# open-genome/dna

Measured on AMD Instinct MI355X. Metric: MLM sequences/sec, DNABERT-2-117M seq_len=512, at 1/2/4/8 MI355X, higher is better.
Workload: dtype bf16

## Files before the change

dna_amd/_native.py:

```python
import ctypes
import os
import re

import torch

_HERE = os.path.dirname(os.path.abspath(__file__))
LIB_PATH = os.environ.get("DNA_AMD_LIB", os.path.join(_HERE, "lib", "libdna_amd.so"))
HEADER = os.path.join(os.path.dirname(_HERE), "include", "dna_amd.h")

F32, BF16, F16 = 0, 1, 2
ACT_NONE, ACT_GELU, ACT_SIGMOID = 0, 1, 2
DCONV_PLAIN, DCONV_GATE, DCONV_MAIN_MUL, DCONV_MAIN_ADD = 0, 1, 2, 3
CLS_REGRESSION, CLS_SINGLE_LABEL, CLS_MULTI_LABEL = 0, 1, 2

_vp, _i, _u64, _f, _sz = ctypes.c_void_p, ctypes.c_int, ctypes.c_uint64, ctypes.c_float, ctypes.c_size_t
_i64 = ctypes.c_int64

_SIGS = {
    "dna_abi_version": (_i, []),
    "dna_abi_revision": (_i, []),
    "dna_last_error": (ctypes.c_char_p, []),
    "dna_attn_fwd": (_i, [_vp, _vp, _vp, _i, _i, _i, _i, _i, _f, _vp, _vp, _vp]),
    "dna_attn_bwd": (_i, [_vp, _vp, _vp, _vp, _vp, _vp, _i, _i, _i, _i, _i, _f, _vp, _vp, _vp]),
    "dna_attn_bwd_ex": (_i, [_vp, _vp, _vp, _vp, _vp, _vp, _i, _i, _i, _i, _i, _f, _vp, _vp, _vp, _vp]),
    "dna_attn_bwd_var": (_i, [_vp, _vp, _vp, _vp, _vp, _vp, _i, _i, _i, _i, _i, _f, _vp, _vp, _vp, _i, _vp]),
    "dna_attn_dbias_part_rows": (_i, [_i, _i]),
    "dna_attn_varlen_fwd": (_i, [_vp, _vp, _vp, _vp, _i, _i, _i, _i, _i, _i, _f, _vp, _vp, _vp]),
    "dna_attn_varlen_bwd_workspace": (_sz, [_i, _i, _i, _i]),
    "dna_attn_varlen_bwd": (_i, [_vp, _vp, _vp, _vp, _vp, _vp, _vp, _i, _i, _i, _i, _i, _i, _f, _vp,
                                 _vp, _vp]),
    "dna_flash_lse_rows": (_i, [_i]),
    "dna_flash_fwd": (_i, [_vp, _i, _vp, _i, _i, _i64, _i64, _i64, _i, _i, _i, _i, _i, _f, _vp, _vp, _vp]),
    "dna_flash_bwd": (_i, [_vp, _i, _vp, _i, _i, _i64, _i64, _i64, _vp, _vp, _vp, _i, _i, _i, _i, _i,
                           _f, _vp, _vp, _vp]),
    "dna_colsum_f32": (_i, [_vp, _i, _i, _vp, _i, _vp]),
    "dna_colsum_bf16_workspace": (_sz, [_i, _i]),
    "dna_colsum_bf16": (_i, [_vp, _i, _i, _vp, _i, _vp, _sz, _vp]),
    "dna_flip_rows": (_i, [_vp, _i, _i, _sz, _vp, _vp]),
    "dna_causal_conv1d_fwd": (_i, [_vp, _sz, _i, _vp, _vp, _i, _i, _i, _i, _i, _vp, _vp]),
    "dna_causal_conv1d_part_rows": (_sz, [_i, _i]),
    "dna_causal_conv1d_bwd": (_i, [_vp, _sz, _i, _vp, _vp, _vp, _i, _i, _i, _i, _i, _vp, _sz, _vp, _vp]),
    "dna_hyena_shortconv_fwd": (_i, [_vp, _i, _vp, _vp, _i, _i, _i, _i, _i, _vp, _vp, _vp]),
    "dna_hyena_shortconv_part_elems": (_sz, [_i, _i, _i, _i, _i]),
    "dna_hyena_shortconv_bwd": (_i, [_vp, _i, _vp, _vp, _i, _i, _i, _i, _i, _vp, _vp, _vp, _vp, _vp]),
    "dna_hyena_gate_out_fwd": (_i, [_vp, _vp, _i, _i, _i, _i, _sz, _vp, _vp]),
    "dna_hyena_gate_out_bwd": (_i, [_vp, _vp, _vp, _i, _i, _i, _i, _sz, _vp, _vp, _vp]),
    "dna_hyena_modulate_t_fwd": (_i, [_vp, _i, _vp, _vp, _f, _i, _i, _i, _vp, _vp]),
    "dna_hyena_modulate_t_bwd": (_i, [_vp, _vp, _vp, _f, _i, _i, _i, _vp, _i, _vp]),
    "dna_hyena_filter_part_elems": (_i, [_i, _i, _i, _i]),
    "dna_hyena_filter_part_stride": (_i, [_i, _i, _i]),
    "dna_hyena_filter_fwd": (_i, [_vp, _vp, _vp, _vp, _vp, _i, _vp, _vp, _vp, _vp, _f, _i, _i, _i, _i,
                                  _vp, _vp]),
    "dna_hyena_filter_bwd": (_i, [_vp, _vp, _vp, _vp, _vp, _i, _vp, _vp, _vp, _vp, _f, _i, _i, _i, _i,
                                  _vp, _vp, _vp, _vp]),
    "dna_hyena_filter_finish": (_i, [_vp, _i, _i, _i, _vp, _vp]),
    "dna_ln_fwd": (_i, [_vp, _i, _vp, _i, _f, _u64, _u64, _vp, _vp, _vp, _i, _i, _f, _vp, _vp,
                        _vp, _vp, _vp]),
    "dna_ln_bwd_workspace": (_sz, [_i, _i]),
    "dna_ln_bwd": (_i, [_vp, _vp, _vp, _i, _vp, _i, _f, _u64, _u64, _vp, _vp, _vp, _vp, _i, _i,
                        _vp, _vp, _vp, _vp, _vp, _vp, _sz, _vp]),
    "dna_ln_bwd_from_y": (_i, [_vp, _vp, _vp, _i, _f, _u64, _u64, _vp, _vp, _vp, _i, _i, _vp,
                               _vp, _vp, _vp, _vp, _vp, _sz, _vp]),
    "dna_ln_bwd_from_y_acc": (_i, [_vp, _vp, _vp, _i, _f, _u64, _u64, _vp, _vp, _vp, _i, _i, _vp,
                                   _vp, _vp, _vp, _vp, _vp, _sz, _vp]),
    "dna_ln_from_y_check": (_i, [_vp, _vp, _vp, _vp, _i, _f, _f, _f, _f, _vp, _vp]),
    "dna_add_ln_fwd": (_i, [_vp, _i, _vp, _vp, _vp, _i, _i, _f, _i, _vp, _vp, _vp, _vp, _vp, _vp]),
    "dna_add_ln_bwd": (_i, [_vp, _vp, _vp, _vp, _i, _vp, _vp, _vp, _vp, _i, _i, _i, _vp, _vp, _vp,
                            _vp, _vp, _sz, _vp]),
    "dna_rms_fwd": (_i, [_vp, _i, _vp, _i, _i, _f, _vp, _vp, _vp, _vp]),
    "dna_rms_bwd": (_i, [_vp, _vp, _vp, _i, _vp, _vp, _i, _i, _vp, _vp, _vp, _sz, _vp]),
    "dna_embed_ln_fwd": (_i, [_vp, _vp, _vp, _vp, _vp, _i, _i, _i, _f, _f, _u64, _u64, _vp, _vp,
                              _vp, _vp, _vp]),
    "dna_embed_ln_bwd": (_i, [_vp, _vp, _vp, _vp, _vp, _vp, _vp, _vp, _i, _i, _i, _i, _f, _u64,
                              _u64, _vp, _vp, _vp, _vp, _vp, _sz, _vp]),
    "dna_embed_ln_bwd_rows": (_i, [_vp, _vp, _vp, _vp, _vp, _vp, _vp, _vp, _i, _i, _i, _f, _u64,
                                   _u64, _vp, _vp, _vp, _vp, _vp, _sz, _vp]),
    "dna_embed_grad_segsum_workspace": (_sz, [_i, _i]),
    "dna_embed_grad_segsum": (_i, [_vp, _vp, _vp, _i, _i, _i, _i, _vp, _vp, _sz, _vp]),
    "dna_sum_slices_accum": (_i, [_vp, _i, _sz, _vp, _vp]),
    "dna_sum_slices": (_i, [_vp, _i, _sz, _vp, _vp]),
    "dna_geglu_fwd": (_i, [_vp, _i, _i, _i, _f, _u64, _u64, _vp, _vp, _vp]),
    "dna_geglu_bwd": (_i, [_vp, _vp, _i, _i, _i, _vp, _vp]),
    "dna_linear_fwd": (_i, [_vp, _vp, _vp, _i, _i, _i, _vp, _vp]),
# ... 146 lines not shown
```

dna_amd/bert_layers.py:

```python
import math
from dataclasses import dataclass
from typing import Optional, Tuple

import torch
import torch.nn as nn

from . import functional as DF
from .config import BertConfig, alibi_slopes

try:
    from transformers.modeling_outputs import MaskedLMOutput
except Exception:
    @dataclass
    class MaskedLMOutput:
        loss: Optional[torch.Tensor] = None
        logits: Optional[object] = None
        hidden_states: Optional[object] = None
        attentions: Optional[object] = None

        def __getitem__(self, i):
            return (self.loss, self.logits)[i]

try:
    from transformers.modeling_outputs import SequenceClassifierOutput
# ... 140 lines not shown
        return self._lpt_provider(p)

    def _linear(self, x, w, b=None, geglu=None):
        return DF.linear(x, w, self._lp(w), b, w_lpt=self._lp_t(w), geglu=geglu)

    def _check_inputs(self, input_ids, token_type_ids, attention_mask):
        if input_ids is None:
            raise ValueError("Must specify input_ids (inputs_embeds is not supported)")
        if token_type_ids is not None and bool((token_type_ids != 0).any()):
            raise NotImplementedError("token_type_ids other than 0 (the MLM path never sets them)")
        if attention_mask is not None:
            if not torch.equal(attention_mask.bool(), input_ids != self.config.pad_token_id_mask):
                raise NotImplementedError("attention_mask must equal input_ids != [PAD]")

    def encode(self, input_ids: torch.Tensor, last_rows: Optional[torch.Tensor] = None,
               packed: Optional["PackedIndex"] = None):
        cfg = self.config
        bert = self._bert_model()
        b, S0 = input_ids.shape
        bf16 = self.precision == "bf16"
        S = S0
        if packed is not None:
            packed.check(input_ids)
            input_ids = input_ids.reshape(-1).index_select(0, packed.indices)
            if last_rows is not None:
                last_rows = packed.row_of.index_select(0, last_rows)
        elif bf16 and S0 % 64:
            S = (S0 + 63) // 64 * 64
            input_ids = torch.nn.functional.pad(input_ids, (0, S - S0), value=cfg.pad_token_id_mask)
            if last_rows is not None:
                last_rows = torch.div(last_rows, S0, rounding_mode="floor") * S + last_rows % S0
        T = b * S if packed is None else packed.total
        H = cfg.num_attention_heads
        train = self.training
        rng = self.dropout_rng
        p_hidden = cfg.hidden_dropout_prob if train else 0.0
        if cfg.attention_probs_dropout_prob and train:
            raise NotImplementedError("attention-probability dropout (reference default 0.0)")
        eps = cfg.layer_norm_eps
        ids = input_ids.reshape(-1)
        key_valid = None if packed is not None else (ids != cfg.pad_token_id_mask).to(torch.uint8)

        emb = bert.embeddings
        seed, off = rng.take(T * cfg.hidden_size) if p_hidden else (0, 0)
        x32, xb = DF.EmbeddingLN.apply(ids, emb.word_embeddings.weight,
                                       emb.token_type_embeddings.weight, emb.LayerNorm.weight,
                                       emb.LayerNorm.bias, eps, p_hidden, seed, off, True, bf16)
        xin = xb if bf16 else x32
        slopes = bert.encoder.alibi_slopes
        L = len(bert.encoder.layer)
        for i, layer in enumerate(bert.encoder.layer):
            att = layer.attention
            qkv = self._linear(xin, att.self.Wqkv.weight, att.self.Wqkv.bias)
            if packed is not None:
                ctx = DF.alibi_attention_varlen(qkv, packed, slopes, H)
            else:
                ctx = DF.alibi_attention(qkv, key_valid, slopes, b, S, H,
                                         bias_grad=att.self.Wqkv.bias is not None)
            res = x32
            if i == L - 1 and last_rows is not None:
                ctx = ctx.index_select(0, last_rows)
                res = x32.index_select(0, last_rows)
            n = ctx.shape[0]
            out = att.output
            h = self._linear(ctx, out.dense.weight)
            seed, off = rng.take(n * cfg.hidden_size) if p_hidden else (0, 0)
            y32, yb = DF.FusedLayerNorm.apply(h, out.dense.bias, res, out.LayerNorm.weight,
                                              out.LayerNorm.bias, eps, 0, p_hidden, seed, off,
                                              True, bf16)
            mlp = layer.mlp
            seed, off = rng.take(n * cfg.intermediate_size) if p_hidden else (0, 0)
            g = self._linear(yb if bf16 else y32, mlp.gated_layers.weight,
                             geglu=(p_hidden, seed, off))
            wo_lp, wo_lpt = self._lp(mlp.wo.weight), self._lp_t(mlp.wo.weight)
            if DF.geglu_out_fused_ok(g, wo_lp, wo_lpt):
                o = DF.geglu_out(g, p_hidden, seed, off, mlp.wo.weight, wo_lp, wo_lpt)
            else:
                a = DF.GeGLU.apply(g, p_hidden, seed, off)
                o = DF.linear(a, mlp.wo.weight, wo_lp, None, w_lpt=wo_lpt)
            x32, xb = DF.FusedLayerNorm.apply(o, mlp.wo.bias, y32, mlp.layernorm.weight,
                                              mlp.layernorm.bias, eps, 0, 0.0, 0, 0, True, bf16)
            xin = xb if bf16 else x32
        if L == 0 and last_rows is not None:
            x32, xin = x32.index_select(0, last_rows), xin.index_select(0, last_rows)
        if packed is None and last_rows is None and S != S0:
            d = x32.shape[1]
            x32 = x32.view(b, S, d)[:, :S0].reshape(b * S0, d)
            xin = xin.view(b, S, d)[:, :S0].reshape(b * S0, d)
        return x32, xin


class BertModel(nn.Module, _HipEncoder):

    def __init__(self, config, add_pooling_layer=False, precision: str = "bf16",
                 init_weights: bool = True):
        super().__init__()
        config = BertConfig.from_any(config)
        self.config = config
        self.embeddings = BertEmbeddings(config)
        self.encoder = BertEncoder(config)
        self.pooler = BertPooler(config) if add_pooling_layer else None
        self._init_hip_encoder(precision)
        if init_weights:
            _init_bert_weights(self, config.initializer_range)
            _tag_projections(self.encoder)

    def _bert_model(self):
        return self

    def forward(self, input_ids, token_type_ids=None, attention_mask=None, position_ids=None,
                output_all_encoded_layers=False, masked_tokens_mask=None, packed=None, **kwargs):
        if output_all_encoded_layers or masked_tokens_mask is not None:
            raise NotImplementedError("BertModel.forward: last layer only, no masked_tokens_mask "
                                      "(the MLM subset path is BertForMaskedLM.mlm_logits)")
# ... 271 lines not shown
```

dna_amd/functional.py:

```python
import math
import os
import warnings

import torch
import torch.nn as nn
import torch.nn.functional as F

from . import _native as N
from .flat import raw_writes

_DT = {torch.float32: N.F32, torch.bfloat16: N.BF16}


def _dt(t):
    try:
        return _DT[t.dtype]
    except KeyError:
        raise TypeError(f"dna_amd: unsupported dtype {t.dtype} (fp32 / bf16 only)")


def _gpu(*ts):
    for t in ts:
        if t is not None and not t.is_cuda:
            raise RuntimeError("dna_amd ops run on the GPU only (no CPU fallback); "
# ... 521 lines not shown
                           + 2 * x.element_size()) + 4)
        with _timed("rms_bwd", nbytes, "byte"):
            N.call("dna_rms_bwd", _p(dy), _p(dyb), x.data_ptr(), _dt(x), gamma.data_ptr(),
                   rstd.data_ptr(), n, d, dx.data_ptr(), dg.data_ptr(), ws.data_ptr(), nws,
                   N.stream_ptr())
        return dx, dg, None, None, None


class AlibiAttention(torch.autograd.Function):

    @staticmethod
    def forward(ctx, qkv, key_valid, slopes, b, S, H, scale, bias_grad=False):
        _gpu(qkv, key_valid, slopes)
        qkv = qkv.contiguous()
        T = qkv.shape[0]
        D = qkv.shape[1] // (3 * H)
        out = torch.empty(T, H * D, device=qkv.device, dtype=qkv.dtype)
        lse = torch.empty(b, H, S, device=qkv.device, dtype=torch.float32)
        with _timed("attn_fwd", 4.0 * b * H * S * S * D):
            N.call("dna_attn_fwd", qkv.data_ptr(), _p(key_valid), slopes.data_ptr(), b, S, H, D,
                   _dt(qkv), scale, out.data_ptr(), lse.data_ptr(), N.stream_ptr())
        ctx.save_for_backward(qkv, out, lse, key_valid, slopes)
        ctx.cfg = (b, S, H, D, scale)
        ctx.bias_grad = bias_grad and qkv.dtype == torch.bfloat16
        return out

    @staticmethod
    def backward(ctx, dout):
        qkv, out, lse, key_valid, slopes = ctx.saved_tensors
        b, S, H, D, scale = ctx.cfg
        dqkv = torch.empty_like(qkv)
        delta = torch.empty(b * H * S, device=qkv.device, dtype=torch.float32)
        dout = dout.contiguous()
        part = None
        if ctx.bias_grad:
            rows = N.lib().dna_attn_dbias_part_rows(b, S)
            part = torch.empty(rows, qkv.shape[1], device=qkv.device, dtype=torch.float32)
        with _timed("attn_bwd", 10.0 * b * H * S * S * D):
            N.call("dna_attn_bwd_ex", qkv.data_ptr(), out.data_ptr(), dout.data_ptr(),
                   lse.data_ptr(), _p(key_valid), slopes.data_ptr(), b, S, H, D, _dt(qkv), scale,
                   dqkv.data_ptr(), delta.data_ptr(), _p(part), N.stream_ptr())
        if part is not None:
            colsum = torch.empty(qkv.shape[1], device=qkv.device, dtype=torch.float32)
            N.call("dna_colsum_f32", part.data_ptr(), part.shape[0], part.shape[1],
                   colsum.data_ptr(), 0, N.stream_ptr())
            dqkv._dna_colsum = colsum
        return dqkv, None, None, None, None, None, None, None


def alibi_attention(qkv, key_valid, slopes, b, S, H, scale=None, bias_grad=False):
    D = qkv.shape[1] // (3 * H)
    return AlibiAttention.apply(qkv, key_valid, slopes, b, S, H,
                                scale if scale is not None else 1.0 / math.sqrt(D), bias_grad)


class AlibiAttentionVarlen(torch.autograd.Function):

    @staticmethod
    def forward(ctx, qkv, cu_seqlens, positions, slopes, nseq, max_seqlen, sq_sum, H, scale):
        _gpu(qkv, cu_seqlens, positions, slopes)
        qkv = qkv.contiguous()
        T = qkv.shape[0]
        D = qkv.shape[1] // (3 * H)
        out = torch.empty(T, H * D, device=qkv.device, dtype=qkv.dtype)
        lse = torch.empty(H, T, device=qkv.device, dtype=torch.float32)
        with _timed("attn_varlen_fwd", 4.0 * H * sq_sum * D):
            N.call("dna_attn_varlen_fwd", qkv.data_ptr(), cu_seqlens.data_ptr(), _p(positions),
                   slopes.data_ptr(), nseq, T, max_seqlen, H, D, _dt(qkv), scale, out.data_ptr(),
                   lse.data_ptr(), N.stream_ptr())
        ctx.save_for_backward(qkv, out, lse, cu_seqlens, positions, slopes)
        ctx.cfg = (nseq, max_seqlen, sq_sum, H, D, scale)
        return out

    @staticmethod
    def backward(ctx, dout):
        qkv, out, lse, cu_seqlens, positions, slopes = ctx.saved_tensors
        nseq, max_seqlen, sq_sum, H, D, scale = ctx.cfg
        T = qkv.shape[0]
        dqkv = torch.empty_like(qkv)
        nws = N.lib().dna_attn_varlen_bwd_workspace(nseq, T, max_seqlen, H)
        ws = torch.empty(nws, device=qkv.device, dtype=torch.uint8)
        dout = dout.contiguous()
        with _timed("attn_varlen_bwd", 10.0 * H * sq_sum * D):
            N.call("dna_attn_varlen_bwd", qkv.data_ptr(), out.data_ptr(), dout.data_ptr(),
                   lse.data_ptr(), cu_seqlens.data_ptr(), _p(positions), slopes.data_ptr(), nseq, T,
                   max_seqlen, H, D, _dt(qkv), scale, dqkv.data_ptr(), ws.data_ptr(),
                   N.stream_ptr())
        return dqkv, None, None, None, None, None, None, None, None


def _check_varlen_index(T, cu_seqlens, positions, nseq):
    if cu_seqlens.dtype != torch.int32 or cu_seqlens.numel() != nseq + 1 or \
            not cu_seqlens.is_contiguous():
        raise ValueError(f"cu_seqlens must be contiguous int32 [{nseq + 1}], got "
                         f"{cu_seqlens.dtype} {tuple(cu_seqlens.shape)}")
    if positions is not None and (positions.dtype != torch.int32 or positions.numel() != T
                                  or not positions.is_contiguous()):
        raise ValueError(f"positions must be contiguous int32 [{T}], got {positions.dtype} "
                         f"{tuple(positions.shape)}")


def alibi_attention_varlen(qkv, packed, slopes, H, scale=None):
    T = qkv.shape[0]
    D = qkv.shape[1] // (3 * H)
    if packed.total != T:
        raise ValueError(f"alibi_attention_varlen: qkv has {T} rows, the index {packed.total}")
# ... 1040 lines not shown
```

include/dna_amd.h:

```cpp
#ifndef DNA_AMD_H
#define DNA_AMD_H

#include <stddef.h>
#include <stdint.h>

#ifdef __cplusplus
extern "C" {
#endif

#define DNA_AMD_ABI_VERSION 1
#define DNA_AMD_ABI_REVISION 5

enum dna_status {
  DNA_OK = 0,
  DNA_ERR_INVALID = 1,
  DNA_ERR_HIP = 2,
  DNA_ERR_UNSUPPORTED = 3,
  DNA_ERR_IO = 4,
  DNA_ERR_NOMEM = 5
};

enum dna_dtype { DNA_F32 = 0, DNA_BF16 = 1, DNA_F16 = 2 };
enum dna_act { DNA_ACT_NONE = 0, DNA_ACT_GELU = 1, DNA_ACT_SIGMOID = 2  };

int dna_abi_version(void);
int dna_abi_revision(void);
const char* dna_last_error(void);

int dna_attn_fwd(const void* qkv, const uint8_t* key_valid, const float* slopes, int batch,
                 int seqlen, int heads, int head_dim, int dtype, float softmax_scale, void* out,
                 float* lse, void* stream);

int dna_flash_lse_rows(int seqlen);
int dna_flash_fwd(const void* qkv, int dtype, const void* bias, int bias_dtype, int bias_type,
                  long long bias_sb, long long bias_sh, long long bias_sq, int batch, int seqlen,
                  int heads, int head_dim, int causal, float softmax_scale, void* out, float* lse,
                  void* stream);
int dna_flash_bwd(const void* qkv, int dtype, const void* bias, int bias_dtype, int bias_type,
                  long long bias_sb, long long bias_sh, long long bias_sq, const void* out,
                  const void* dout, const float* lse, int batch, int seqlen, int heads,
                  int head_dim, int causal, float softmax_scale, float* delta, void* dqkv,
                  void* stream);

int dna_attn_bwd(const void* qkv, const void* out, const void* dout, const float* lse,
                 const uint8_t* key_valid, const float* slopes, int batch, int seqlen, int heads,
                 int head_dim, int dtype, float softmax_scale, void* dqkv, float* delta_ws,
                 void* stream);
int dna_attn_bwd_ex(const void* qkv, const void* out, const void* dout, const float* lse,
                    const uint8_t* key_valid, const float* slopes, int batch, int seqlen, int heads,
                    int head_dim, int dtype, float softmax_scale, void* dqkv, float* delta_ws,
                    float* dbias_part, void* stream);
int dna_attn_bwd_var(const void* qkv, const void* out, const void* dout, const float* lse,
                     const uint8_t* key_valid, const float* slopes, int batch, int seqlen, int heads,
                     int head_dim, int dtype, float softmax_scale, void* dqkv, float* delta_ws,
                     float* dbias_part, int nw, void* stream);
int dna_attn_dbias_part_rows(int batch, int seqlen);

int dna_attn_varlen_fwd(const void* qkv, const int* cu_seqlens, const int* positions,
                        const float* slopes, int nseq, int total_rows, int max_seqlen, int heads,
                        int head_dim, int dtype, float softmax_scale, void* out, float* lse,
                        void* stream);
size_t dna_attn_varlen_bwd_workspace(int nseq, int total_rows, int max_seqlen, int heads);
int dna_attn_varlen_bwd(const void* qkv, const void* out, const void* dout, const float* lse,
                        const int* cu_seqlens, const int* positions, const float* slopes, int nseq,
                        int total_rows, int max_seqlen, int heads, int head_dim, int dtype,
                        float softmax_scale, void* dqkv, void* workspace, void* stream);

int dna_ln_fwd(const void* x, int x_dtype, const float* bias, int act, float p_drop,
               uint64_t seed, uint64_t offset, const float* residual, const float* gamma,
               const float* beta, int rows, int cols, float eps, float* y, void* y_bf16,
               float* mean, float* rstd, void* stream);

size_t dna_ln_bwd_workspace(int rows, int cols);
int dna_ln_bwd(const float* dy, const void* dy_bf16, const void* x, int x_dtype,
               const float* bias, int act, float p_drop, uint64_t seed, uint64_t offset,
               const float* residual, const float* gamma, const float* mean, const float* rstd,
               int rows, int cols, float* dresidual, void* dx, float* dgamma, float* dbeta,
               float* dbias, void* workspace, size_t workspace_bytes, void* stream);
int dna_ln_bwd_from_y(const float* dy, const void* dy_bf16, const float* y, int x_dtype,
                      float p_drop, uint64_t seed, uint64_t offset, const float* gamma,
                      const float* beta, const float* rstd, int rows, int cols, float* dresidual,
                      void* dx, float* dgamma, float* dbeta, float* dbias, void* workspace,
                      size_t workspace_bytes, void* stream);
int dna_ln_bwd_from_y_acc(const float* dy, const void* dy_bf16, const float* y, int x_dtype,
                          float p_drop, uint64_t seed, uint64_t offset, const float* gamma,
                          const float* beta, const float* rstd, int rows, int cols,
                          float* dresidual, void* dx, float* dgamma, float* dbeta, float* dbias,
                          void* workspace, size_t workspace_bytes, void* stream);
int dna_ln_from_y_check(const float* base, const int64_t* gamma_off, const int64_t* beta_off,
                        const int* cols, int npairs, float max_ratio, float min_gamma,
                        float margin, float shrink, int* ok, void* stream);

int dna_add_ln_fwd(const void* x, int x_dtype, const float* residual, const float* gamma,
                   const float* beta, int rows, int cols, float eps, int rms, float* sum, float* y,
                   void* y_bf16, float* mean, float* rstd, void* stream);
int dna_add_ln_bwd(const float* dy, const void* dy_bf16, const float* dsum, const void* x,
                   int x_dtype, const float* residual, const float* gamma, const float* mean,
                   const float* rstd, int rows, int cols, int rms, float* dresidual, void* dx,
                   float* dgamma, float* dbeta, void* workspace, size_t workspace_bytes,
                   void* stream);

int dna_rms_fwd(const void* x, int x_dtype, const float* gamma, int rows, int cols, float eps,
                float* y, void* y_bf16, float* rstd, void* stream);
int dna_rms_bwd(const float* dy, const void* dy_bf16, const void* x, int x_dtype,
                const float* gamma, const float* rstd, int rows, int cols, void* dx,
                float* dgamma, void* workspace, size_t workspace_bytes, void* stream);

int dna_embed_ln_fwd(const int64_t* ids, const float* word_emb, const float* type_row,
                     const float* gamma, const float* beta, int rows, int cols, int vocab,
                     float eps, float p_drop, uint64_t seed, uint64_t offset, float* y,
                     void* y_bf16, float* mean, float* rstd, void* stream);

int dna_embed_ln_bwd(const float* dy, const void* dy_bf16, const int64_t* ids,
                     const float* word_emb, const float* type_row, const float* gamma,
                     const float* mean, const float* rstd, int rows, int cols, int vocab,
                     int padding_idx, float p_drop, uint64_t seed, uint64_t offset,
                     float* dword_emb, float* dtype_row, float* dgamma, float* dbeta,
                     void* workspace, size_t workspace_bytes, void* stream);

// ... 280 lines not shown
```

Baseline: 2498.

## Compute last-layer attention only for masked query rows

Adds subset attention forward and backward kernels that evaluate the last encoder layer's attention only for the query rows later used by the MLM loss (last_rows), rather than running full attention and index_selecting afterwards. The backward computes dq for the subset rows only, zeroes dq for the other rows, and computes dK/dV from the subset queries. The intent is to cut last-layer attention FLOPs, roughly in proportion to the masked fraction. It adds new kernels, searchsorted-based per-sequence offsets and an env toggle, and assumes rows are sorted.

```diff
diff --git a/dna_amd/_native.py b/dna_amd/_native.py
--- a/dna_amd/_native.py
+++ b/dna_amd/_native.py
@@ -29,6 +29,10 @@
     "dna_attn_varlen_bwd_workspace": (_sz, [_i, _i, _i, _i]),
     "dna_attn_varlen_bwd": (_i, [_vp, _vp, _vp, _vp, _vp, _vp, _vp, _i, _i, _i, _i, _i, _i, _f, _vp,
                                  _vp, _vp]),
+    "dna_attn_subset_fwd": (_i, [_vp, _vp, _vp, _vp, _vp, _i, _i, _i, _i, _i, _i, _f, _vp, _vp, _vp]),
+    "dna_attn_subset_bwd": (_i, [_vp, _vp, _vp, _vp, _vp, _vp, _vp, _vp, _i, _i, _i, _i, _i, _i, _f,
+                                 _vp, _vp, _vp, _vp]),
+    "dna_attn_subset_dbias_part_rows": (_i, [_i, _i]),
     "dna_flash_lse_rows": (_i, [_i]),
     "dna_flash_fwd": (_i, [_vp, _i, _vp, _i, _i, _i64, _i64, _i64, _i, _i, _i, _i, _i, _f, _vp, _vp, _vp]),
     "dna_flash_bwd": (_i, [_vp, _i, _vp, _i, _i, _i64, _i64, _i64, _vp, _vp, _vp, _i, _i, _i, _i, _i,
diff --git a/dna_amd/bert_layers.py b/dna_amd/bert_layers.py
--- a/dna_amd/bert_layers.py
+++ b/dna_amd/bert_layers.py
@@ -216,14 +216,21 @@
         for i, layer in enumerate(bert.encoder.layer):
             att = layer.attention
             qkv = self._linear(xin, att.self.Wqkv.weight, att.self.Wqkv.bias)
+            last = i == L - 1 and last_rows is not None
+            subset = (last and bf16 and packed is None and qkv.shape[1] == 3 * H * 64
+                      and DF.attention_subset_enabled())
             if packed is not None:
                 ctx = DF.alibi_attention_varlen(qkv, packed, slopes, H)
+            elif subset:
+                ctx = DF.alibi_attention_subset(qkv, key_valid, slopes, last_rows, b, S, H,
+                                                bias_grad=att.self.Wqkv.bias is not None)
             else:
                 ctx = DF.alibi_attention(qkv, key_valid, slopes, b, S, H,
                                          bias_grad=att.self.Wqkv.bias is not None)
             res = x32
-            if i == L - 1 and last_rows is not None:
-                ctx = ctx.index_select(0, last_rows)
+            if last:
+                if not subset:
+                    ctx = ctx.index_select(0, last_rows)
                 res = x32.index_select(0, last_rows)
             n = ctx.shape[0]
             out = att.output
diff --git a/dna_amd/csrc/attention_subset.hip b/dna_amd/csrc/attention_subset.hip
--- /dev/null
+++ b/dna_amd/csrc/attention_subset.hip
@@ -0,0 +1,617 @@
+#include <limits.h>
+
+#include "common.h"
+
+namespace dna {
+namespace attn_subset {
+
+constexpr int D = 64;
+constexpr int KT = 64;
+constexpr int LDW = D + 8;
+constexpr int NWQ = 4;
+constexpr int NWK = 4;
+constexpr int QT = 128;
+constexpr int MAX_S = 32768;
+constexpr float LOG2E = 1.4426950408889634f;
+constexpr float LN2 = 0.6931471805599453f;
+constexpr float PAD_BIAS = -10000.0f;
+
+typedef __attribute__((ext_vector_type(4))) short s16x4;
+
+__device__ __forceinline__ f32x16 mfma(bf16x8 a, bf16x8 b, f32x16 c) {
+  return __builtin_amdgcn_mfma_f32_32x32x16_bf16(a, b, c, 0, 0, 0);
+}
+__device__ __forceinline__ float ex2(float x) { return __builtin_amdgcn_exp2f(x); }
+__device__ __forceinline__ float pair_sum(float x) { return x + __shfl_xor(x, 32, 64); }
+__device__ __forceinline__ float pair_max(float x) { return fmaxf(x, __shfl_xor(x, 32, 64)); }
+
+__device__ __forceinline__ float half_sum16(const f32x16& v, int ql) {
+  float a8[8], a4[4], a2[2];
+  bool up = ql & 16;
+#pragma unroll
+  for (int i = 0; i < 8; ++i)
+    a8[i] = (up ? v[i + 8] : v[i]) + __shfl_xor(up ? v[i] : v[i + 8], 16, 64);
+  up = ql & 8;
+#pragma unroll
+  for (int i = 0; i < 4; ++i)
+    a4[i] = (up ? a8[i + 4] : a8[i]) + __shfl_xor(up ? a8[i] : a8[i + 4], 8, 64);
+  up = ql & 4;
+#pragma unroll
+  for (int i = 0; i < 2; ++i)
+    a2[i] = (up ? a4[i + 2] : a4[i]) + __shfl_xor(up ? a4[i] : a4[i + 2], 4, 64);
+  up = ql & 2;
+  const float a1 = (up ? a2[1] : a2[0]) + __shfl_xor(up ? a2[0] : a2[1], 2, 64);
+  return a1 + __shfl_xor(a1, 1, 64);
+}
+
+__device__ __forceinline__ constexpr int aoff(int r) { return (r & 3) + 8 * (r >> 2); }
+
+__device__ __forceinline__ bf16x8 tr_operand(const bf16* tile, int row0, int dt, int lane) {
+  const int g16 = lane >> 4, i16 = lane & 15;
+  const int row = row0 + 4 * (g16 >> 1) + (i16 >> 2);
+  const int col = 32 * dt + 16 * (g16 & 1) + 4 * (i16 & 3);
+  const s16x4 lo = __builtin_amdgcn_ds_read_tr16_b64_v4i16(
+      (__attribute__((address_space(3))) s16x4*)(tile + row * LDW + col));
+  const s16x4 hi = __builtin_amdgcn_ds_read_tr16_b64_v4i16(
+      (__attribute__((address_space(3))) s16x4*)(tile + (row + 8) * LDW + col));
+  const bf16x4 a = __builtin_bit_cast(bf16x4, lo), b = __builtin_bit_cast(bf16x4, hi);
+  return bf16x8{a[0], a[1], a[2], a[3], b[0], b[1], b[2], b[3]};
+}
+
+struct SeqRows {
+  int cu0, nrows;
+};
+__device__ __forceinline__ SeqRows seq_rows(const int* __restrict__ cu, int n, int R) {
+  const int a = min(max(cu[n], 0), R);
+  const int b = min(max(cu[n + 1], a), R);
+  return {a, b - a};
+}
+__device__ __forceinline__ int row_at(const long long* __restrict__ rows, int k, int T) {
+  const long long r = rows[k];
+  return (int)(r < 0 ? 0 : (r < T ? r : T - 1));
+}
+
+struct KVRegs {
+  bf16x8 k[2], v[2];
+  float bias;
+};
+__device__ __forceinline__ void kv_fetch(KVRegs& t, const bf16* __restrict__ kbase, size_t ld,
+                                         size_t hd, const uint8_t* __restrict__ kvalid, int k0,
+                                         int tid) {
+  const int r = tid >> 3, ch = (tid & 7) * 8;
+#pragma unroll
+  for (int i = 0; i < 2; ++i) {
+    const bf16* src = kbase + (size_t)(k0 + r + 32 * i) * ld + ch;
+    t.k[i] = *reinterpret_cast<const bf16x8*>(src);
+    t.v[i] = *reinterpret_cast<const bf16x8*>(src + hd);
+  }
+  t.bias = (tid < KT && kvalid && !kvalid[k0 + tid]) ? PAD_BIAS * LOG2E : 0.f;
+}
+__device__ __forceinline__ void kv_store(const KVRegs& t, bf16* Ks, bf16* Vs, float* kbs, int tid) {
+  const int r = tid >> 3, ch = (tid & 7) * 8;
+#pragma unroll
+  for (int i = 0; i < 2; ++i) {
+    *reinterpret_cast<bf16x8*>(Ks + (r + 32 * i) * LDW + ch) = t.k[i];
+    *reinterpret_cast<bf16x8*>(Vs + (r + 32 * i) * LDW + ch) = t.v[i];
+  }
+  if (tid < KT) kbs[tid] = t.bias;
+}
+
+__global__ __launch_bounds__(NWQ * 64) void fwd_kernel(
+    const bf16* __restrict__ qkv, const uint8_t* __restrict__ key_valid,
+    const float* __restrict__ slopes, const long long* __restrict__ rows,
+    const int* __restrict__ cu, int S, int H, int T, int R, float c, bf16* __restrict__ out,
+    float* __restrict__ lse) {
+  __shared__ __attribute__((aligned(16))) bf16 Ks[KT * LDW];
+  __shared__ __attribute__((aligned(16))) bf16 Vs[KT * LDW];
+  __shared__ __attribute__((aligned(16))) float kbs[KT];
+  const int tid = threadIdx.x, wave = tid >> 6, lane = tid & 63, ql = lane & 31, hh = lane >> 5;
+  const int n = blockIdx.x / H, h = blockIdx.x % H;
+  const SeqRows sq = seq_rows(cu, n, R);
+  if (sq.nrows == 0) return;
+  const size_t ld = (size_t)3 * H * D, hd = (size_t)H * D;
+  const bf16* kbase = qkv + (size_t)n * S * ld + hd + h * D;
+  const uint8_t* kvalid = key_valid ? key_valid + (size_t)n * S : nullptr;
+  const float slope2 = slopes[h] * LOG2E;
+
+  for (int q0 = 0; q0 < sq.nrows; q0 += NWQ * 32) {
+    const bool active = q0 + 32 * wave < sq.nrows;
+    const int qi = q0 + 32 * wave + ql;
+    const bool qok = qi < sq.nrows;
+    const int kq = sq.cu0 + min(qi, sq.nrows - 1);
+    const int qrow = row_at(rows, kq, T);
+    const float qpos = (float)(qrow % S);
+    bf16x8 qf[4];
+#pragma unroll
+    for (int s = 0; s < 4; ++s)
+      qf[s] = *reinterpret_cast<const bf16x8*>(qkv + (size_t)qrow * ld + h * D + 16 * s + 8 * hh);
+    float m = -INFINITY, l = 0.f;
+    f32x16 o[2];
+#pragma unroll
+    for (int r = 0; r < 16; ++r) { o[0][r] = 0.f; o[1][r] = 0.f; }
+
+    KVRegs nxt;
+    kv_fetch(nxt, kbase, ld, hd, kvalid, 0, tid);
+    for (int k0 = 0; k0 < S; k0 += KT) {
+      __syncthreads();
+      kv_store(nxt, Ks, Vs, kbs, tid);
+      __syncthreads();
+      if (k0 + KT < S) kv_fetch(nxt, kbase, ld, hd, kvalid, k0 + KT, tid);
+      if (!active) continue;
+      f32x16 sa[2];
+      float mx = -INFINITY;
+#pragma unroll
+      for (int kh = 0; kh < 2; ++kh) {
+#pragma unroll
+        for (int r = 0; r < 16; ++r) sa[kh][r] = 0.f;
+#pragma unroll
+        for (int s = 0; s < 4; ++s) {
+          const bf16x8 ak =
+              *reinterpret_cast<const bf16x8*>(Ks + (kh * 32 + ql) * LDW + 16 * s + 8 * hh);
+          sa[kh] = mfma(ak, qf[s], sa[kh]);
+        }
+#pragma unroll
+        for (int g = 0; g < 4; ++g) {
+          const int ko = kh * 32 + 8 * g + 4 * hh;
+          const f32x4 kb = *reinterpret_cast<const f32x4*>(kbs + ko);
+#pragma unroll
+          for (int e = 0; e < 4; ++e) {
+            const float dist = fabsf(qpos - (float)(k0 + ko + e));
+            const float x = fmaf(sa[kh][4 * g + e], c, fmaf(-slope2, dist, kb[e]));
+            sa[kh][4 * g + e] = x;
+            mx = fmaxf(mx, x);
+          }
+        }
+      }
+      const float mn = fmaxf(m, pair_max(mx));
+      const float alpha = ex2(m - mn);
+      m = mn;
+      float psum = 0.f;
+      bf16x8 pb[2][2];
+#pragma unroll
+      for (int kh = 0; kh < 2; ++kh)
+#pragma unroll
+        for (int r = 0; r < 16; ++r) {
+          const float p = ex2(sa[kh][r] - mn);
+          psum += p;
+          pb[kh][r >> 3][r & 7] = (bf16)p;
+        }
+      l = fmaf(l, alpha, psum);
+#pragma unroll
+      for (int r = 0; r < 16; ++r) { o[0][r] *= alpha; o[1][r] *= alpha; }
+#pragma unroll
+      for (int kh = 0; kh < 2; ++kh)
+#pragma unroll
+        for (int s = 0; s < 2; ++s)
+#pragma unroll
+          for (int dt = 0; dt < 2; ++dt)
+            o[dt] = mfma(tr_operand(Vs, kh * 32 + 16 * s, dt, lane), pb[kh][s], o[dt]);
+    }
+    if (active) {
+      const float lt = pair_sum(l);
+      if (qok) {
+        const float inv = 1.f / lt;
+        bf16* orow = out + (size_t)kq * hd + h * D;
+#pragma unroll
+        for (int dt = 0; dt < 2; ++dt)
+#pragma unroll
+          for (int g = 0; g < 4; ++g) {
+            bf16x4 v;
+#pragma unroll
+            for (int e = 0; e < 4; ++e) v[e] = (bf16)(o[dt][4 * g + e] * inv);
+            *reinterpret_cast<bf16x4*>(orow + 32 * dt + 8 * g + 4 * hh) = v;
+          }
+        if (hh == 0) lse[(size_t)h * R + kq] = (m + __log2f(lt)) * LN2;
+      }
+    }
+  }
+}
+
+template <bool DBE>
+__global__ __launch_bounds__(NWQ * 64) void dq_kernel(
+    const bf16* __restrict__ qkv, const bf16* __restrict__ out, const bf16* __restrict__ dout,
+    const float* __restrict__ lse, float* __restrict__ delta,
+    const uint8_t* __restrict__ key_valid, const float* __restrict__ slopes,
+    const long long* __restrict__ rows, const int* __restrict__ cu, int S, int H, int T, int R,
+    float c, float scale, bf16* __restrict__ dqkv, float* __restrict__ dbias_part) {
+  __shared__ __attribute__((aligned(16))) bf16 Ks[KT * LDW];
+  __shared__ __attribute__((aligned(16))) bf16 Vs[KT * LDW];
+  __shared__ __attribute__((aligned(16))) float kbs[KT];
+  __shared__ float red[NWQ][D];
+  extern __shared__ uint8_t in_subset[];
+  const int tid = threadIdx.x, wave = tid >> 6, lane = tid & 63, ql = lane & 31, hh = lane >> 5;
+  const int n = blockIdx.x / H, h = blockIdx.x % H;
+  const SeqRows sq = seq_rows(cu, n, R);
+  const size_t ld = (size_t)3 * H * D, hd = (size_t)H * D;
+  const bf16* kbase = qkv + (size_t)n * S * ld + hd + h * D;
+  const uint8_t* kvalid = key_valid ? key_valid + (size_t)n * S : nullptr;
+  const float slope2 = slopes[h] * LOG2E;
+
+  for (int j = tid; j < S; j += NWQ * 64) in_subset[j] = 0;
+  if (DBE) red[wave][lane] = 0.f;
+  __syncthreads();
+  for (int k = tid; k < sq.nrows; k += NWQ * 64) {
+    const int r = row_at(rows, sq.cu0 + k, T);
+    if (r / S == n) in_subset[r % S] = 1;
+  }
+  __syncthreads();
+  {
+    bf16x8 z;
+#pragma unroll
+    for (int j = 0; j < 8; ++j) z[j] = (bf16)0.f;
+    bf16* qdst = dqkv + (size_t)n * S * ld + h * D;
+    for (int idx = tid; idx < S * 8; idx += NWQ * 64)
+      if (!in_subset[idx >> 3])
+        *reinterpret_cast<bf16x8*>(qdst + (size_t)(idx >> 3) * ld + (idx & 7) * 8) = z;
+  }
+
+  for (int q0 = 0; q0 < sq.nrows; q0 += NWQ * 32) {
+    const bool active = q0 + 32 * wave < sq.nrows;
+    const int qi = q0 + 32 * wave + ql;
+    const int kq = sq.cu0 + min(qi, sq.nrows - 1);
+    const int qrow = row_at(rows, kq, T);
+    const bool qok = qi < sq.nrows && qrow / S == n;
+    const float qpos = (float)(qrow % S);
+    bf16x8 qf[4], df[4];
+    float acc = 0.f;
+    {
+      const size_t orow = (size_t)kq * hd + h * D;
+#pragma unroll
+      for (int s = 0; s < 4; ++s) {
+        qf[s] = *reinterpret_cast<const bf16x8*>(qkv + (size_t)qrow * ld + h * D + 16 * s + 8 * hh);
+        df[s] = *reinterpret_cast<const bf16x8*>(dout + orow + 16 * s + 8 * hh);
+        const bf16x8 o8 = *reinterpret_cast<const bf16x8*>(out + orow + 16 * s + 8 * hh);
+#pragma unroll
+        for (int j = 0; j < 8; ++j) acc = fmaf((float)df[s][j], (float)o8[j], acc);
+      }
+    }
+    const float dl = pair_sum(acc);
+    const float lse2 = lse[(size_t)h * R + kq] * LOG2E;
+    if (active && qi < sq.nrows && hh == 0) delta[(size_t)h * R + kq] = dl;
+    f32x16 dq[2];
+#pragma unroll
+    for (int r = 0; r < 16; ++r) { dq[0][r] = 0.f; dq[1][r] = 0.f; }
+
+    KVRegs nxt;
+    kv_fetch(nxt, kbase, ld, hd, kvalid, 0, tid);
+    for (int k0 = 0; k0 < S; k0 += KT) {
+      __syncthreads();
+      kv_store(nxt, Ks, Vs, kbs, tid);
+      __syncthreads();
+      if (k0 + KT < S) kv_fetch(nxt, kbase, ld, hd, kvalid, k0 + KT, tid);
+      if (!active) continue;
+#pragma unroll
+      for (int kh = 0; kh < 2; ++kh) {
+        f32x16 sa, pa;
+#pragma unroll
+        for (int r = 0; r < 16; ++r) { sa[r] = 0.f; pa[r] = -dl; }
+#pragma unroll
+        for (int s = 0; s < 4; ++s) {
+          const int off = (kh * 32 + ql) * LDW + 16 * s + 8 * hh;
+          sa = mfma(*reinterpret_cast<const bf16x8*>(Ks + off), qf[s], sa);
+          pa = mfma(*reinterpret_cast<const bf16x8*>(Vs + off), df[s], pa);
+        }
+        bf16x8 db[2];
+#pragma unroll
+        for (int g = 0; g < 4; ++g) {
+          const int ko = kh * 32 + 8 * g + 4 * hh;
+          const f32x4 kb = *reinterpret_cast<const f32x4*>(kbs + ko);
+#pragma unroll
+          for (int e = 0; e < 4; ++e) {
+            const int r = 4 * g + e;
+            const float dist = fabsf(qpos - (float)(k0 + ko + e));
+            const float x = fmaf(sa[r], c, fmaf(-slope2, dist, kb[e])) - lse2;
+            db[r >> 3][r & 7] = (bf16)(ex2(x) * pa[r]);
+          }
+        }
+#pragma unroll
+        for (int s = 0; s < 2; ++s)
+#pragma unroll
+          for (int dt = 0; dt < 2; ++dt)
+            dq[dt] = mfma(tr_operand(Ks, kh * 32 + 16 * s, dt, lane), db[s], dq[dt]);
+      }
+    }
+    if (active) {
+      if (qok) {
+        bf16* row = dqkv + (size_t)qrow * ld + h * D;
+#pragma unroll
+        for (int dt = 0; dt < 2; ++dt)
+#pragma unroll
+          for (int g = 0; g < 4; ++g) {
+            bf16x4 v;
+#pragma unroll
+            for (int e = 0; e < 4; ++e) v[e] = (bf16)(dq[dt][4 * g + e] * scale);
+            *reinterpret_cast<bf16x4*>(row + 32 * dt + 8 * g + 4 * hh) = v;
+          }
+      }
+      if (DBE) {
+#pragma unroll
+        for (int dt = 0; dt < 2; ++dt) {
+          f32x16 t;
+#pragma unroll
+          for (int r = 0; r < 16; ++r) t[r] = qok ? dq[dt][r] * scale : 0.f;
+          const float v = half_sum16(t, ql);
+          if ((ql & 1) == 0) red[wave][32 * dt + aoff(ql >> 1) + 4 * hh] += v;
+        }
+      }
+    }
+  }
+  if (DBE) {
+    __syncthreads();
+    if (tid < D)
+      dbias_part[(size_t)n * ld + h * D + tid] =
+          (red[0][tid] + red[1][tid]) + (red[2][tid] + red[3][tid]);
+  }
+}
+
+__device__ __forceinline__ void stage_queries(
+    bf16* Qs, bf16* Os, float* qpos, float* ql2, float* qdl, const bf16* __restrict__ qkv,
+    const bf16* __restrict__ dout, const float* __restrict__ lse, const float* __restrict__ delta,
+    const long long* __restrict__ rows, SeqRows sq, int s0, int S, int T, int R, size_t ld,
+    size_t hd, int h, int tid) {
+  const int nr = min(QT, sq.nrows - s0), nr32 = (nr + 31) & ~31;
+  constexpr int NI = QT * 8 / (NWK * 64);
+  const int ch = (tid & 7) * 8;
+  int qrow[NI];
+  bf16x8 a[NI], b[NI];
+#pragma unroll
+  for (int i = 0; i < NI; ++i) {
+    const int r = (tid >> 3) + (NWK * 8) * i;
+    qrow[i] = r < nr ? row_at(rows, sq.cu0 + s0 + r, T) : 0;
+  }
+#pragma unroll
+  for (int i = 0; i < NI; ++i) {
+    const int r = (tid >> 3) + (NWK * 8) * i;
+#pragma unroll
+    for (int j = 0; j < 8; ++j) { a[i][j] = (bf16)0.f; b[i][j] = (bf16)0.f; }
+    if (r < nr) {
+      a[i] = *reinterpret_cast<const bf16x8*>(qkv + (size_t)qrow[i] * ld + h * D + ch);
+      b[i] = *reinterpret_cast<const bf16x8*>(dout + (size_t)(sq.cu0 + s0 + r) * hd + h * D + ch);
+    }
+  }
+#pragma unroll
+  for (int i = 0; i < NI; ++i) {
+    const int r = (tid >> 3) + (NWK * 8) * i;
+    if (r < nr32) {
+      *reinterpret_cast<bf16x8*>(Qs + r * LDW + ch) = a[i];
+      *reinterpret_cast<bf16x8*>(Os + r * LDW + ch) = b[i];
+    }
+  }
+  if (tid < nr32) {
+    const bool in = tid < nr;
+    const int k = sq.cu0 + s0 + min(tid, nr - 1);
+    qpos[tid] = in ? (float)(row_at(rows, k, T) % S) : 0.f;
+    ql2[tid] = in ? lse[(size_t)h * R + k] * LOG2E : 0.f;
+    qdl[tid] = in ? delta[(size_t)h * R + k] : 0.f;
+  }
+}
+
+template <bool DBE>
+__global__ __launch_bounds__(NWK * 64) void dkdv_kernel(
+    const bf16* __restrict__ qkv, const bf16* __restrict__ dout, const float* __restrict__ lse,
+    const float* __restrict__ delta, const uint8_t* __restrict__ key_valid,
+    const float* __restrict__ slopes, const long long* __restrict__ rows,
+    const int* __restrict__ cu, int S, int H, int T, int R, float c, float scale,
+    bf16* __restrict__ dqkv, float* __restrict__ dbias_part) {
+  __shared__ __attribute__((aligned(16))) bf16 Qs[QT * LDW];
+  __shared__ __attribute__((aligned(16))) bf16 Os[QT * LDW];
+  __shared__ __attribute__((aligned(16))) float qpos[QT], ql2[QT], qdl[QT];
+  __shared__ float red[NWK][2][D];
+  __shared__ __attribute__((aligned(16))) bf16 Tb[NWK * 32 * LDW];
+  const int tid = threadIdx.x, wave = tid >> 6, lane = tid & 63, kl = lane & 31, hh = lane >> 5;
+  const int n = blockIdx.x / H, h = blockIdx.x % H;
+  const SeqRows sq = seq_rows(cu, n, R);
+  const size_t ld = (size_t)3 * H * D, hd = (size_t)H * D;
+  const float slope2 = slopes[h] * LOG2E;
+  if (DBE) { red[wave][0][lane] = 0.f; red[wave][1][lane] = 0.f; }
+  const bf16* kvbase = qkv + (size_t)n * S * ld + h * D + 8 * hh;
+  const uint8_t* kvalid = key_valid ? key_valid + (size_t)n * S : nullptr;
+  bf16x8 kf[4], vf[4];
+  float kbias;
+  {
+    const int kj = min(32 * wave + kl, S - 1);
+#pragma unroll
+    for (int s = 0; s < 4; ++s) {
+      kf[s] = *reinterpret_cast<const bf16x8*>(kvbase + (size_t)kj * ld + hd + 16 * s);
+      vf[s] = *reinterpret_cast<const bf16x8*>(kvbase + (size_t)kj * ld + 2 * hd + 16 * s);
+    }
+    kbias = (kvalid && !kvalid[kj]) ? PAD_BIAS * LOG2E : 0.f;
+  }
+  bf16* tb = Tb + wave * 32 * LDW;
+  const bool once = sq.nrows <= QT;
+  if (once) {
+    stage_queries(Qs, Os, qpos, ql2, qdl, qkv, dout, lse, delta, rows, sq, 0, S, T, R, ld, hd, h,
+                  tid);
+    __syncthreads();
+  }
+
+  for (int kp = 0; kp < S; kp += NWK * 32) {
+    const int kbase = kp + 32 * wave;
+    const bool active = kbase < S;
+    f32x16 dk[2], dv[2];
+    const float kpos = (float)min(kbase + kl, S - 1);
+#pragma unroll
+    for (int r = 0; r < 16; ++r) { dk[0][r] = 0.f; dk[1][r] = 0.f; dv[0][r] = 0.f; dv[1][r] = 0.f; }
+
+    for (int s0 = 0; s0 < sq.nrows; s0 += QT) {
+      if (!once) {
+        __syncthreads();
+        stage_queries(Qs, Os, qpos, ql2, qdl, qkv, dout, lse, delta, rows, sq, s0, S, T, R, ld, hd,
+                      h, tid);
+        __syncthreads();
+      }
+      if (!active) continue;
+      const int nq = min(QT, sq.nrows - s0);
+#pragma unroll 1
+      for (int q0 = 0; q0 < nq; q0 += 32) {
+        f32x16 sa, pa;
+#pragma unroll
+        for (int r = 0; r < 16; ++r) { sa[r] = 0.f; pa[r] = 0.f; }
+#pragma unroll
+        for (int s = 0; s < 4; ++s) {
+          const int off = (q0 + kl) * LDW + 16 * s + 8 * hh;
+          sa = mfma(*reinterpret_cast<const bf16x8*>(Qs + off), kf[s], sa);
+          pa = mfma(*reinterpret_cast<const bf16x8*>(Os + off), vf[s], pa);
+        }
+        bf16x8 pb[2], sb[2];
+#pragma unroll
+        for (int g = 0; g < 4; ++g) {
+          const int qo = q0 + 8 * g + 4 * hh;
+          const f32x4 qp = *reinterpret_cast<const f32x4*>(qpos + qo);
+          const f32x4 l4 = *reinterpret_cast<const f32x4*>(ql2 + qo);
+          const f32x4 d4 = *reinterpret_cast<const f32x4*>(qdl + qo);
+#pragma unroll
+          for (int e = 0; e < 4; ++e) {
+            const int r = 4 * g + e;
+            const float dist = fabsf(qp[e] - kpos);
+            const float x = fmaf(sa[r], c, fmaf(-slope2, dist, kbias)) - l4[e];
+            const float p = qo + e < nq ? ex2(x) : 0.f;
+            pb[r >> 3][r & 7] = (bf16)p;
+            sb[r >> 3][r & 7] = (bf16)(p * (pa[r] - d4[e]));
+          }
+        }
+#pragma unroll
+        for (int s = 0; s < 2; ++s)
+#pragma unroll
+          for (int dt = 0; dt < 2; ++dt) {
+            dv[dt] = mfma(tr_operand(Os, q0 + 16 * s, dt, lane), pb[s], dv[dt]);
+            dk[dt] = mfma(tr_operand(Qs, q0 + 16 * s, dt, lane), sb[s], dk[dt]);
+          }
+      }
+    }
+    if (!active) continue;
+    const bool more = kbase + NWK * 32 < S;
+    bf16x8 nk[4], nv[4];
+    float nbias = 0.f;
+    if (more) {
+      const int kj = kbase + NWK * 32 + kl;
+#pragma unroll
+      for (int s = 0; s < 4; ++s) {
+        nk[s] = *reinterpret_cast<const bf16x8*>(kvbase + (size_t)kj * ld + hd + 16 * s);
+        nv[s] = *reinterpret_cast<const bf16x8*>(kvbase + (size_t)kj * ld + 2 * hd + 16 * s);
+      }
+      nbias = (kvalid && !kvalid[kj]) ? PAD_BIAS * LOG2E : 0.f;
+    }
+#pragma unroll
+    for (int ts = 0; ts < 2; ++ts) {
+#pragma unroll
+      for (int dt = 0; dt < 2; ++dt)
+#pragma unroll
+        for (int g = 0; g < 4; ++g) {
+          bf16x4 v;
+#pragma unroll
+          for (int e = 0; e < 4; ++e)
+            v[e] = ts == 0 ? (bf16)(dk[dt][4 * g + e] * scale) : (bf16)dv[dt][4 * g + e];
+          *reinterpret_cast<bf16x4*>(tb + kl * LDW + 32 * dt + 8 * g + 4 * hh) = v;
+        }
+      bf16* dst = dqkv + ((size_t)n * S + kbase) * ld + (1 + ts) * hd + h * D + (lane & 7) * 8;
+#pragma unroll
+      for (int i = 0; i < 4; ++i) {
+        const int row = (lane >> 3) + 8 * i;
+        *reinterpret_cast<bf16x8*>(dst + (size_t)row * ld) =
+            *reinterpret_cast<const bf16x8*>(tb + row * LDW + (lane & 7) * 8);
+      }
+    }
+    if (DBE) {
+#pragma unroll
+      for (int dt = 0; dt < 2; ++dt) {
+        const float sk = half_sum16(dk[dt], kl) * scale, sv = half_sum16(dv[dt], kl);
+        if ((kl & 1) == 0) {
+          const int d = 32 * dt + aoff(kl >> 1) + 4 * hh;
+          red[wave][0][d] += sk;
+          red[wave][1][d] += sv;
+        }
+      }
+    }
+    if (more) {
+#pragma unroll
+      for (int s = 0; s < 4; ++s) { kf[s] = nk[s]; vf[s] = nv[s]; }
+      kbias = nbias;
+    }
+  }
+  if (DBE) {
+    __syncthreads();
+    if (tid < 2 * D) {
+      const int ts = tid >> 6, d = tid & 63;
+      float sum = 0.f;
+#pragma unroll
+      for (int w = 0; w < NWK; ++w) sum += red[w][ts][d];
+      dbias_part[(size_t)n * ld + (1 + ts) * hd + h * D + d] = sum;
+    }
+  }
+}
+
+}
+}
+
+using namespace dna;
+using namespace dna::attn_subset;
+
+static int check_common(const void* qkv, const float* slopes, const int64_t* rows,
+                        const int* cu_rows, int batch, int seqlen, int heads, int head_dim,
+                        int nrows, int dtype, const char* fn) {
+  DNA_CHECK_ARG(qkv && slopes && cu_rows, "%s: null pointer", fn);
+  DNA_CHECK_ARG(batch > 0 && seqlen > 0 && heads > 0 && nrows >= 0,
+                "%s: bad shape b=%d S=%d H=%d R=%d", fn, batch, seqlen, heads, nrows);
+  DNA_CHECK_ARG(rows || nrows == 0, "%s: null rows with R=%d", fn, nrows);
+  DNA_CHECK_ARG((long long)batch * seqlen <= INT_MAX && (long long)batch * heads <= INT_MAX,
+                "%s: b=%d S=%d H=%d is too large", fn, batch, seqlen, heads);
+  if (head_dim != D || dtype != DNA_BF16 || seqlen % KT != 0 || seqlen > MAX_S) {
+    set_error("%s: needs bf16, head_dim 64 and seqlen %% 64 == 0 up to %d (got dtype %d, "
+              "head_dim %d, seqlen %d)", fn, MAX_S, dtype, head_dim, seqlen);
+    return DNA_ERR_UNSUPPORTED;
+  }
+  return DNA_OK;
+}
+
+extern "C" int dna_attn_subset_fwd(const void* qkv, const uint8_t* key_valid, const float* slopes,
+                                   const int64_t* rows, const int* cu_rows, int batch, int seqlen,
+                                   int heads, int head_dim, int nrows, int dtype,
+                                   float softmax_scale, void* out_sub, float* lse_sub,
+                                   void* stream) {
+  int st = check_common(qkv, slopes, rows, cu_rows, batch, seqlen, heads, head_dim, nrows, dtype,
+                        "dna_attn_subset_fwd");
+  if (st) return st;
+  if (nrows == 0) return DNA_OK;
+  DNA_CHECK_ARG(out_sub && lse_sub, "dna_attn_subset_fwd: null output");
+  hipLaunchKernelGGL(fwd_kernel, dim3(batch * heads), dim3(NWQ * 64), 0, as_stream(stream),
+                     (const bf16*)qkv, key_valid, slopes, (const long long*)rows, cu_rows, seqlen,
+                     heads, batch * seqlen, nrows, softmax_scale * LOG2E, (bf16*)out_sub, lse_sub);
+  DNA_LAUNCH_CHECK("dna_attn_subset_fwd");
+  return DNA_OK;
+}
+
+extern "C" int dna_attn_subset_bwd(const void* qkv, const void* out_sub, const void* dout_sub,
+                                   const float* lse_sub, const uint8_t* key_valid,
+                                   const float* slopes, const int64_t* rows, const int* cu_rows,
+                                   int batch, int seqlen, int heads, int head_dim, int nrows,
+                                   int dtype, float softmax_scale, void* dqkv, float* delta_ws,
+                                   float* dbias_part, void* stream) {
+  int st = check_common(qkv, slopes, rows, cu_rows, batch, seqlen, heads, head_dim, nrows, dtype,
+                        "dna_attn_subset_bwd");
+  if (st) return st;
+  DNA_CHECK_ARG(dqkv, "dna_attn_subset_bwd: null dqkv");
+  DNA_CHECK_ARG(nrows == 0 || (out_sub && dout_sub && lse_sub && delta_ws),
+                "dna_attn_subset_bwd: null pointer");
+  hipStream_t s = as_stream(stream);
+  const dim3 grid(batch * heads);
+  const long long* r64 = (const long long*)rows;
+  const int T = batch * seqlen;
+  const float c = softmax_scale * LOG2E;
+  const auto dq = dbias_part ? dq_kernel<true> : dq_kernel<false>;
+  const auto dkdv = dbias_part ? dkdv_kernel<true> : dkdv_kernel<false>;
+  hipLaunchKernelGGL(dq, grid, dim3(NWQ * 64), (size_t)seqlen, s, (const bf16*)qkv,
+                     (const bf16*)out_sub, (const bf16*)dout_sub, lse_sub, delta_ws, key_valid,
+                     slopes, r64, cu_rows, seqlen, heads, T, nrows, c, softmax_scale, (bf16*)dqkv,
+                     dbias_part);
+  hipLaunchKernelGGL(dkdv, grid, dim3(NWK * 64), 0, s, (const bf16*)qkv, (const bf16*)dout_sub,
+                     lse_sub, delta_ws, key_valid, slopes, r64, cu_rows, seqlen, heads, T, nrows, c,
+                     softmax_scale, (bf16*)dqkv, dbias_part);
+  DNA_LAUNCH_CHECK("dna_attn_subset_bwd");
+  return DNA_OK;
+}
+
+extern "C" int dna_attn_subset_dbias_part_rows(int batch, int seqlen) {
+  (void)seqlen;
+  return batch > 0 ? batch : 0;
+}
diff --git a/dna_amd/functional.py b/dna_amd/functional.py
--- a/dna_amd/functional.py
+++ b/dna_amd/functional.py
@@ -597,6 +597,80 @@
     D = qkv.shape[1] // (3 * H)
     return AlibiAttention.apply(qkv, key_valid, slopes, b, S, H,
                                 scale if scale is not None else 1.0 / math.sqrt(D), bias_grad)
+
+
+class AlibiAttentionSubset(torch.autograd.Function):
+
+    @staticmethod
+    def forward(ctx, qkv, key_valid, slopes, rows, cu_rows, b, S, H, scale, bias_grad=False):
+        _gpu(qkv, key_valid, slopes, rows, cu_rows)
+        qkv = qkv.contiguous()
+        D = qkv.shape[1] // (3 * H)
+        R = rows.numel()
+        out = torch.empty(R, H * D, device=qkv.device, dtype=qkv.dtype)
+        lse = torch.empty(H, R, device=qkv.device, dtype=torch.float32)
+        with _timed("attn_sub_fwd", 4.0 * H * R * S * D):
+            N.call("dna_attn_subset_fwd", qkv.data_ptr(), _p(key_valid), slopes.data_ptr(),
+                   _p(rows), cu_rows.data_ptr(), b, S, H, D, R, _dt(qkv), scale, _p(out), _p(lse),
+                   N.stream_ptr())
+        ctx.save_for_backward(qkv, out, lse, key_valid, slopes, rows, cu_rows)
+        ctx.cfg = (b, S, H, D, scale)
+        ctx.bias_grad = bias_grad
+        return out
+
+    @staticmethod
+    def backward(ctx, dout):
+        qkv, out, lse, key_valid, slopes, rows, cu_rows = ctx.saved_tensors
+        b, S, H, D, scale = ctx.cfg
+        R = rows.numel()
+        dqkv = torch.empty_like(qkv)
+        delta = torch.empty(H * R, device=qkv.device, dtype=torch.float32)
+        dout = dout.contiguous()
+        part = None
+        if ctx.bias_grad:
+            nrow = N.lib().dna_attn_subset_dbias_part_rows(b, S)
+            part = torch.empty(nrow, qkv.shape[1], device=qkv.device, dtype=torch.float32)
+        with _timed("attn_sub_bwd", 10.0 * H * R * S * D):
+            N.call("dna_attn_subset_bwd", qkv.data_ptr(), _p(out), _p(dout), _p(lse),
+                   _p(key_valid), slopes.data_ptr(), _p(rows), cu_rows.data_ptr(), b, S, H, D, R,
+                   _dt(qkv), scale, dqkv.data_ptr(), _p(delta), _p(part), N.stream_ptr())
+        if part is not None:
+            colsum = torch.empty(qkv.shape[1], device=qkv.device, dtype=torch.float32)
+            N.call("dna_colsum_f32", part.data_ptr(), part.shape[0], part.shape[1],
+                   colsum.data_ptr(), 0, N.stream_ptr())
+            dqkv._dna_colsum = colsum
+        return dqkv, None, None, None, None, None, None, None, None, None
+
+
+def attention_subset_enabled():
+    v = os.environ.get("DNA_ATTN_SUBSET", "1")
+    if v not in ("0", "1"):
+        raise ValueError(f"DNA_ATTN_SUBSET={v!r}: 0 or 1")
+    return v == "1"
+
+
+def subset_cu_rows(rows, b, S):
+    bounds = torch.arange(b + 1, device=rows.device, dtype=rows.dtype) * S
+    return torch.searchsorted(rows, bounds).to(torch.int32)
+
+
+def alibi_attention_subset(qkv, key_valid, slopes, rows, b, S, H, scale=None, bias_grad=False,
+                           cu_rows=None):
+    D = qkv.shape[1] // (3 * H)
+    if qkv.dtype != torch.bfloat16 or D != 64 or S % 64 or qkv.shape[0] != b * S:
+        raise ValueError(f"alibi_attention_subset: needs bf16 qkv [b*S, 3*H*64] with S % 64 == 0, "
+                         f"got {qkv.dtype} {tuple(qkv.shape)} b={b} S={S} H={H}")
+    if rows.dtype != torch.int64 or rows.dim() != 1:
+        raise ValueError(f"rows must be int64 [R], got {rows.dtype} {tuple(rows.shape)}")
+    rows = rows.contiguous()
+    if cu_rows is None:
+        cu_rows = subset_cu_rows(rows, b, S)
+    elif cu_rows.dtype != torch.int32 or cu_rows.numel() != b + 1 or not cu_rows.is_contiguous():
+        raise ValueError(f"cu_rows must be contiguous int32 [{b + 1}], got {cu_rows.dtype} "
+                         f"{tuple(cu_rows.shape)}")
+    return AlibiAttentionSubset.apply(qkv, key_valid, slopes, rows, cu_rows, b, S, H,
+                                      scale if scale is not None else 1.0 / math.sqrt(D),
+                                      bias_grad)
 
 
 class AlibiAttentionVarlen(torch.autograd.Function):
diff --git a/include/dna_amd.h b/include/dna_amd.h
--- a/include/dna_amd.h
+++ b/include/dna_amd.h
@@ -9,7 +9,7 @@
 #endif
 
 #define DNA_AMD_ABI_VERSION 1
-#define DNA_AMD_ABI_REVISION 5
+#define DNA_AMD_ABI_REVISION 6
 
 enum dna_status {
   DNA_OK = 0,
@@ -65,6 +65,17 @@
                         const int* cu_seqlens, const int* positions, const float* slopes, int nseq,
                         int total_rows, int max_seqlen, int heads, int head_dim, int dtype,
                         float softmax_scale, void* dqkv, void* workspace, void* stream);
+
+int dna_attn_subset_fwd(const void* qkv, const uint8_t* key_valid, const float* slopes,
+                        const int64_t* rows, const int* cu_rows, int batch, int seqlen, int heads,
+                        int head_dim, int nrows, int dtype, float softmax_scale, void* out_sub,
+                        float* lse_sub, void* stream);
+int dna_attn_subset_bwd(const void* qkv, const void* out_sub, const void* dout_sub,
+                        const float* lse_sub, const uint8_t* key_valid, const float* slopes,
+                        const int64_t* rows, const int* cu_rows, int batch, int seqlen, int heads,
+                        int head_dim, int nrows, int dtype, float softmax_scale, void* dqkv,
+                        float* delta_ws, float* dbias_part, void* stream);
+int dna_attn_subset_dbias_part_rows(int batch, int seqlen);
 
 int dna_ln_fwd(const void* x, int x_dtype, const float* bias, int act, float p_drop,
                uint64_t seed, uint64_t offset, const float* residual, const float* gamma,
```

Measured after the change: 2515, median of 6. About the same (+0.7%).
